# seanwood/gcc-nmf

Measured on NVIDIA H100. Metric: STFT frames/sec (1024-FFT, K=1024) full GCC-NMF pipeline, higher is better.
Workload: dtype f32

## Files before the change

gcc-nmf_b200/csrc/gcc_tc.cu:

```cuda
#include <algorithm>

#include "common.cuh"
#include "tma_gemm_host.cuh"

namespace {

using namespace tgemm_host;

inline float margin_factor(int F) {
  const double per_value = 3.0 / 262144.0 + (1.0 + 3.0 * F / 16.0) / 16777216.0;
  return (float)(2.5 * per_value);
}

__global__ void __launch_bounds__(256)
build_gcc_planes_kernel(const float2* __restrict__ coh, int F, int T, const double2* __restrict__ E, int D, bf16* __restrict__ G, int64_t pitch,
                        int64_t plane) {
  __shared__ float2 Cs[64][33];
  const int f0 = blockIdx.x * 64, t0 = blockIdx.y * 32;
  const int lane = threadIdx.x & 31, w = threadIdx.x >> 5;
  for (int i = w; i < 64; i += 8) {
    const int f = f0 + i, t = t0 + lane;
    Cs[i][lane] = (f < F && t < T) ? coh[(int64_t)f * T + t] : float2{0.f, 0.f};
  }
  __syncthreads();
// ... 26 lines not shown
    }
  }
}

__global__ void split_to_planes_kernel(const float* __restrict__ src, int64_t n, bf16* __restrict__ planes, int64_t plane) {
  const int64_t i = (int64_t)blockIdx.x * blockDim.x + threadIdx.x;
  if (i >= n) return;
  bf16 hi, lo;
  split_bf16(src[i], hi, lo);
  planes[i] = hi;
  planes[plane + i] = lo;
}

struct EpiArgmaxTile {
  static constexpr bool kTileEpilogue = true;
  static constexpr bool kRowReduce = false;
  static constexpr int kRowValues = 0;
  static constexpr bool kPrefetch = false;
  struct State {};
  struct Loaded {};
  int32_t* __restrict__ argmax;
  const float* __restrict__ colsumW;
  int2* __restrict__ list; uint4* __restrict__ candidates; int* __restrict__ count; int capacity;
  int K, T, D; float margin_factor;
  __device__ void prefetch(int, int) const {}
  __device__ void row_values(int, float*) const {}
  __device__ void elem(int, int, float, int) const {}
  __device__ void tile_epilogue(const float* __restrict__ tile, int m0, int n0, int n_valid, int) const {
    const int frames = n_valid / D;
    for (int p = threadIdx.x; p < tgemm::kBM * frames; p += blockDim.x) {
      const int ml = p & (tgemm::kBM - 1), j = p / tgemm::kBM;
      const int m = m0 + ml;
      if (m >= K) continue;
      const float* col = tile + (size_t)(j * D) * tgemm::kBM + ml;
      float best = -INFINITY, second = -INFINITY;
      int idx = 0, nan = 0;
#pragma unroll 8
      for (int d = 0; d < D; ++d) {
        const float x = col[(size_t)d * tgemm::kBM];
        if (x != x) nan = 1;
        if (x > best) { second = best; best = x; idx = d; }
        else if (x > second) second = x;
      }
      const int t = n0 / D + j;
      argmax[(int64_t)m * T + t] = idx;
      const float margin = margin_factor * colsumW[m];
      if (nan || !(best - second > margin)) {
        uint32_t bits[4] = {0u, 0u, 0u, 0u};
        for (int d = 0; d < D; ++d) {
          const float x = col[(size_t)d * tgemm::kBM];
          if (nan || !(best - x > margin)) bits[d >> 5] |= 1u << (d & 31);
        }
        const int slot = atomicAdd(count, 1);
        if (slot < capacity) {
          list[slot] = make_int2(m, t);
          candidates[slot] = make_uint4(bits[0], bits[1], bits[2], bits[3]);
        }
      }
    }
  }
};

constexpr int kPersBN = 256, kPersKB = 32, kPersStages = 4;
constexpr int kPersABytes = 2 * tgemm::kBM * kPersKB * 2;
constexpr int kPersBBytes = 2 * kPersBN * kPersKB * 2;
constexpr int kPersStageBytes = kPersABytes + kPersBBytes;
constexpr int kPersSmem = kPersStages * kPersStageBytes + 256 + 1024;
constexpr int kPersAtomBytes = 2 * kPersKB * 128;

struct ArgmaxPartial {
  float best, second;
  int idx, nan;
  __device__ void scan(float x, int d) {
    if (x != x) nan = 1;
    if (x > best) { second = best; best = x; idx = d; }
    else if (x > second) second = x;
  }
  __device__ void merge_xor(int o) {
    const float ob = __shfl_xor_sync(0xffffffffu, best, o), os = __shfl_xor_sync(0xffffffffu, second, o);
    const int oi = __shfl_xor_sync(0xffffffffu, idx, o), on = __shfl_xor_sync(0xffffffffu, nan, o);
    const bool take = ob > best || (ob == best && oi < idx);
    const float loser = take ? best : ob;
    if (take) { best = ob; idx = oi; }
// ... 585 lines not shown
```

gcc-nmf_b200/csrc/klnmf_tma.cu:

```cuda
#include <algorithm>
#include <mutex>
#include <utility>
#include <vector>

#include "common.cuh"
#include "tma_gemm_host.cuh"

void gccnmf_tmap_cache_free(gccnmf_handle* h) {
  delete h->tmaps;
  h->tmaps = nullptr;
}

namespace {

using namespace tgemm_host;

constexpr int kApplyTile = 32;

struct EpiStoreT {
  struct State {};
  struct Loaded {};
  static constexpr bool kDualN = true;
  static constexpr bool kRowReduce = false;
  static constexpr int kRowValues = 0;
  static constexpr bool kPrefetch = false;
  float* __restrict__ DT; int64_t ld, slab; int M, N; bool vec; bool streaming;
  __device__ void prefetch(int, int) const {}
  __device__ void row_values(int, float*) const {}
  __device__ void init(State&, int, const float*) const {}
  __device__ float4 row_partial(const State&) const { return make_float4(0.f, 0.f, 0.f, 0.f); }
  __device__ void row_total(int, int, float) const {}
  __device__ void elem(int m, int n, float acc, int z) const { DT[(int64_t)z * slab + (int64_t)n * ld + m] = acc; }
  __device__ Loaded load(int, int) const { return Loaded{}; }
  __device__ void store(int m, int n, const float4& acc, const Loaded&, int z, State&) const {
    const int valid = min(4, M - m);
    if (valid <= 0) return;
    if (streaming) store4_streaming(DT + (int64_t)z * slab + (int64_t)n * ld + m, acc, valid, vec);
    else store4(DT + (int64_t)z * slab + (int64_t)n * ld + m, acc, valid, vec);
  }
};

struct EpiRatioPlanes {
  struct State {};
  struct Loaded { float4 vt; };
  static constexpr bool kRowReduce = false;
  static constexpr int kRowValues = 0;
  static constexpr bool kPrefetch = false;
  static constexpr bool kDualN = true;
  static constexpr bool kPreloadOperands = true;
  const float* __restrict__ VT; bf16* __restrict__ RT; int64_t ld, plane; int M, N; bool vec;
  __device__ void prefetch(int, int) const {}
  __device__ void row_values(int, float*) const {}
  __device__ void init(State&, int, const float*) const {}
  __device__ float4 row_partial(const State&) const { return make_float4(0.f, 0.f, 0.f, 0.f); }
  __device__ void row_total(int, int, float) const {}
  __device__ void elem(int m, int n, float acc, int) const {
    bf16 hi, lo;
    split_bf16(VT[(int64_t)n * ld + m] / acc, hi, lo);
    RT[(int64_t)n * ld + m] = hi;
    RT[plane + (int64_t)n * ld + m] = lo;
  }
  __device__ Loaded load(int m, int n) const { return Loaded{load4(VT + (int64_t)n * ld + m, min(4, M - m), vec, 1.f)}; }
  __device__ void store(int m, int n, const float4& acc, const Loaded& l, int, State&) const {
    const int valid = min(4, M - m);
    if (valid <= 0) return;
    const float4 r = make_float4(__fdividef(l.vt.x, acc.x), __fdividef(l.vt.y, acc.y), __fdividef(l.vt.z, acc.z), __fdividef(l.vt.w, acc.w));
    store_planes4(RT + (int64_t)n * ld + m, plane, r, valid, vec);
  }
};

struct EpiUpdateH {
  struct State { float4 rden, rsum; };
  struct Loaded { float4 old; };
  static constexpr bool kRowReduce = true;
  static constexpr int kRowValues = 1;
  static constexpr bool kPrefetch = true;
  __device__ void prefetch(int m, int n) const {
    if (m < M) tgemm::prefetch_l2(HT + (int64_t)n * ld + m);
  }
  float* __restrict__ HT; bf16* __restrict__ HTp; const float* __restrict__ colsum_part; const float* __restrict__ sumsq_part;
  float* __restrict__ rowsum_part; float alpha, eps; int64_t ld, plane; int M, N; int slots; bool vec;
  __device__ void row_values(int m, float* v) const {
    v[0] = 1.f;
// ... 978 lines not shown
```

gcc-nmf_b200/csrc/tma_gemm.cuh:

```cuda
#pragma once
#include <cuda.h>
#include <cuda_bf16.h>
#include <cuda_runtime.h>

#include <cstdint>
#include <type_traits>

#include "gmma_ptx.cuh"

namespace tgemm {

using gmma::mbar_init;
using gmma::mbar_wait;
using gmma::smem_u32;

constexpr int kBM = 128;
constexpr int kMmaWarpgroups = 2;
constexpr int kAuxWarps = 3;
constexpr int kThreads = (1 + kMmaWarpgroups) * 128;
constexpr int kColumnsInFlight = 8;
constexpr int kMaxRowValues = 4;
constexpr int kSmemBudget = 216 * 1024;

__device__ __forceinline__ void mbar_arrive_expect_tx(uint32_t bar, uint32_t bytes) {
  asm volatile("mbarrier.arrive.expect_tx.shared::cta.b64 _, [%0], %1;" ::"r"(bar), "r"(bytes) : "memory");
}
__device__ __forceinline__ void tma_load_3d(uint32_t dst, const CUtensorMap* map, uint32_t bar, int c0, int c1, int c2) {
  asm volatile(
      "cp.async.bulk.tensor.3d.shared::cluster.global.mbarrier::complete_tx::bytes [%0], [%1, {%3, %4, %5}], [%2];"
      ::"r"(dst), "l"(reinterpret_cast<uint64_t>(map)), "r"(bar), "r"(c0), "r"(c1), "r"(c2)
      : "memory");
}
template <bool MULTICAST>
__device__ __forceinline__ void tma_load_3d_mc(uint32_t dst, const CUtensorMap* map, uint32_t bar, int c0, int c1, int c2, uint16_t mask) {
  if (MULTICAST) {
    asm volatile(
        "cp.async.bulk.tensor.3d.shared::cluster.global.mbarrier::complete_tx::bytes.multicast::cluster [%0], [%1, {%3, %4, %5}], [%2], %6;"
        ::"r"(dst), "l"(reinterpret_cast<uint64_t>(map)), "r"(bar), "r"(c0), "r"(c1), "r"(c2), "h"(mask)
        : "memory");
  } else {
    tma_load_3d(dst, map, bar, c0, c1, c2);
  }
}
__device__ __forceinline__ void cluster_sync() {
  asm volatile("barrier.cluster.arrive.release.aligned;" ::: "memory");
  asm volatile("barrier.cluster.wait.acquire.aligned;" ::: "memory");
}
__device__ __forceinline__ float4 ld_cluster_f32x4(const float* local, uint32_t rank) {
  uint32_t remote;
  asm volatile("mapa.shared::cluster.u32 %0, %1, %2;" : "=r"(remote) : "r"(gmma::smem_u32(local)), "r"(rank));
  float4 v;
  asm volatile("ld.shared::cluster.v4.f32 {%0, %1, %2, %3}, [%4];" : "=f"(v.x), "=f"(v.y), "=f"(v.z), "=f"(v.w) : "r"(remote) : "memory");
  return v;
}
__device__ __forceinline__ void tma_prefetch_descriptor(const CUtensorMap* map) {
// ... 18 lines not shown
  const uint32_t hw[4] = {h.x, h.y, h.z, h.w}, lw[4] = {l.x, l.y, l.z, l.w};
#pragma unroll
  for (int i = 0; i < 4; ++i) {
    out[2 * i] = __uint_as_float(hw[i] << 16) + __uint_as_float(lw[i] << 16);
    out[2 * i + 1] = __uint_as_float(hw[i] & 0xFFFF0000u) + __uint_as_float(lw[i] & 0xFFFF0000u);
  }
}

struct PeerSignal {
  unsigned* counters[8];
  int world;
};
__device__ __forceinline__ void signal_peers(const PeerSignal& sig) {
  for (int r = 0; r < sig.world; ++r) asm volatile("red.relaxed.sys.global.add.u32 [%0], %1;" ::"l"(sig.counters[r]), "r"(1u) : "memory");
}

struct PlaneGemmArgs {
  int M, N, Kc;
  int m_tiles;
  int tail_rows;
  int tail_cols;
  int kblocks_per_split;
  int preload;
  int m_fastest;
  int z_cluster;
  const __nv_bfloat16* A; int64_t a_plane, lda;
  const __nv_bfloat16* B; int64_t b_plane, ldb;
  unsigned* done_counter;
  PeerSignal signal;
  unsigned long long* timing;
};


template <int BN, int KB, bool A_MN, bool B_MN, int NACC = 1>
struct Config {
  static_assert(KB == 32 || KB == 64, "k-block of 32 (SWIZZLE_64B K-major rows) or 64 (SWIZZLE_128B)");
  static_assert(BN % 8 == 0 && BN >= 16 && BN * NACC <= 256, "wgmma N (= BN, or 2 BN in the dual-N loop)");
  static constexpr int kAAtoms = kBM / 64;
  static constexpr int kBAtoms = (BN + 63) / 64;
  static constexpr int kAtomBytes = 2 * KB * 128;
  static constexpr int kABytes = 2 * kBM * KB * 2;
  static constexpr int kBBytes = B_MN ? kBAtoms * kAtomBytes : 2 * BN * KB * 2;
  static constexpr int kStageBytes = kABytes + kBBytes;
  static_assert(kABytes % 1024 == 0 && kBBytes % 1024 == 0, "operand blocks must keep 1024-byte alignment");
  static constexpr int kStagesRaw = kSmemBudget / kStageBytes;
  static constexpr int kStages = kStagesRaw > 8 ? 8 : kStagesRaw;
  static_assert(kStages >= 2, "tile too large for a 2-stage pipeline");
  static constexpr int kAccCols = BN * NACC;
  static constexpr int kBarrierBytes = 256;
  static constexpr int kScratchBytes = kMaxRowValues * kBM * 4 + (kThreads / 32) * 32 * 16;
  static constexpr int kTotal = kStages * kStageBytes + kBarrierBytes + kScratchBytes + 1024;
  static_assert(kStages * kStageBytes >= BN * kBM * 4, "the epilogue stages the accumulator tile in the pipeline buffers");
  static_assert(kTotal <= 227 * 1024, "shared memory per CTA");
};

template <int N, int KB, bool A_MN, bool B_MN, bool DUAL>
__device__ __forceinline__ void mma_kblock(float (&acc)[N / 2], uint32_t a_base, uint32_t b_base, uint32_t b_lo_off) {
  constexpr uint32_t kAtom = 2 * KB * 128;
  constexpr uint32_t a_lo_off = A_MN ? KB * 128 : kBM * KB * 2;
  constexpr uint32_t a_step = A_MN ? 2048u : 32u, b_step = B_MN ? 2048u : 32u;
  constexpr uint32_t kKSbo = 8 * KB * 2;
  constexpr uint32_t kKSwizzle = (KB == 32) ? gmma::kSwizzle64B : gmma::kSwizzle128B;
  auto desc = [&](uint32_t addr, bool mn) {
    return mn ? gmma::make_desc(addr, kAtom, 1024, gmma::kSwizzle128B) : gmma::make_desc(addr, 16, kKSbo, kKSwizzle);
  };
#pragma unroll
  for (int kk = 0; kk < KB / 16; ++kk) {
    const uint32_t a_addr = a_base + kk * a_step, b_addr = b_base + kk * b_step;
    const uint64_t a_hi = desc(a_addr, A_MN), a_lo = desc(a_addr + a_lo_off, A_MN);
    const uint64_t b_hi = desc(b_addr, B_MN), b_lo = desc(b_addr + b_lo_off, B_MN);
    if constexpr (DUAL) {
      if (kk > 0) gmma::wgmma_fence();
      gmma::Wgmma<N / 2>::template mma<A_MN, B_MN>(reinterpret_cast<float(&)[N / 4]>(acc), a_lo, b_hi);
      gmma::wgmma_fence();
      gmma::Wgmma<N>::template mma<A_MN, B_MN>(acc, a_hi, b_hi);
      (void)b_lo;
    } else {
      gmma::Wgmma<N>::template mma<A_MN, B_MN>(acc, a_lo, b_hi);
      gmma::Wgmma<N>::template mma<A_MN, B_MN>(acc, a_hi, b_lo);
      gmma::Wgmma<N>::template mma<A_MN, B_MN>(acc, a_hi, b_hi);
    }
  }
}

template <class E, class = void>
struct has_tile_epilogue { static constexpr bool value = false; };
template <class E>
struct has_tile_epilogue<E, decltype((void)E::kTileEpilogue)> { static constexpr bool value = E::kTileEpilogue; };

template <class E, class = void>
struct wants_preload { static constexpr bool value = false; };
template <class E>
struct wants_preload<E, decltype((void)E::kPreloadOperands)> { static constexpr bool value = E::kPreloadOperands; };

template <class E, class = void>
struct wants_dual_n { static constexpr bool value = false; };
template <class E>
struct wants_dual_n<E, decltype((void)E::kDualN)> { static constexpr bool value = E::kDualN; };

template <int BN, int KB, bool A_MN, bool B_MN, int CN, int CM, class Epilogue>
__global__ void __launch_bounds__(kThreads, 1)
plane_gemm_kernel(const __grid_constant__ CUtensorMap map_a, const __grid_constant__ CUtensorMap map_b, PlaneGemmArgs args, Epilogue epi) {
  constexpr bool DUAL = wants_dual_n<Epilogue>::value && !B_MN && 2 * BN <= 256;
  using C = Config<BN, KB, A_MN, B_MN, DUAL ? 2 : 1>;
  constexpr int kCluster = CN * CM;
  static_assert((CN == 1 || CN == 2) && (CM == 1 || CM == 2), "cluster of CN n-tiles x CM m-tiles");
  static_assert(A_MN || (kBM / CN) % 8 == 0, "A row slices keep the swizzle atoms whole");
  static_assert(B_MN || (BN / CM) % 8 == 0, "B row slices keep the swizzle atoms whole");
  extern __shared__ unsigned char smem_dyn[];
  unsigned char* smem = reinterpret_cast<unsigned char*>((reinterpret_cast<uintptr_t>(smem_dyn) + 1023) & ~uintptr_t(1023));

  const int tid = threadIdx.x, warp = tid >> 5, lane = tid & 31;
  const bool mf = args.m_fastest != 0;
  const int tile_n = mf ? (int)blockIdx.y : (int)blockIdx.x;
  const int tile_m = mf ? (int)blockIdx.x : (int)blockIdx.y;
  const int z = blockIdx.z;
  const int n0 = tile_n * BN;
  const int total_kblocks = (args.Kc + KB - 1) / KB;
  const int kb_begin = z * args.kblocks_per_split;
  const int kb_end = min(total_kblocks, kb_begin + args.kblocks_per_split);
  const int num_kb = max(0, kb_end - kb_begin);
  const int cx = (!mf && CN > 1) ? (int)(blockIdx.x % CN) : 0;
  const int cy = (CM > 1) ? tile_m % CM : 0;
  const uint16_t mask_row = (uint16_t)(((1u << CN) - 1u) << (CN * cy));
  const uint16_t mask_col = (uint16_t)((CM > 1 ? ((1u << cx) | (1u << (cx + CN))) : (1u << cx)));

  uint64_t* bars = reinterpret_cast<uint64_t*>(smem + C::kStages * C::kStageBytes);
  uint64_t* full = bars;
  uint64_t* empty = bars + C::kStages;
  float* rowvals = reinterpret_cast<float*>(smem + C::kStages * C::kStageBytes + C::kBarrierBytes);
  float4* red = reinterpret_cast<float4*>(rowvals + kMaxRowValues * kBM);
  float* tile = reinterpret_cast<float*>(smem);
  const int m0 = tile_m * kBM;

  const int cta_linear = blockIdx.x + gridDim.x * (blockIdx.y + gridDim.y * blockIdx.z);
  if (args.timing && tid == 0) {
    args.timing[cta_linear * 8 + 0] = globaltimer_ns();
    args.timing[cta_linear * 8 + 1] = clock64();
  }
  if (tid == 0) {
    for (int s = 0; s < C::kStages; ++s) {
      mbar_init(smem_u32(&full[s]), 1);
      mbar_init(smem_u32(&empty[s]), kMmaWarpgroups * (CN + CM - 1));
    }
    gmma::fence_barrier_init();
    tma_prefetch_descriptor(&map_a);
    tma_prefetch_descriptor(&map_b);
  }
  if (kCluster > 1) cluster_sync();
  else __syncthreads();
  pdl_launch_dependents();
  pdl_wait_prior_grids();

  constexpr int kWarpsAll = kThreads / 32;
  constexpr int kLoadedWords = (int)((sizeof(typename Epilogue::Loaded) + 3) / 4);
  constexpr bool kPreloads = wants_preload<Epilogue>::value && !has_tile_epilogue<Epilogue>::value && !std::is_empty<typename Epilogue::Loaded>::value;
  constexpr int kPreCap = 64 / (kLoadedWords > 0 ? kLoadedWords : 1);
  constexpr int kPre = kPreloads ? ((BN + kWarpsAll - 1) / kWarpsAll < kPreCap ? (BN + kWarpsAll - 1) / kWarpsAll : kPreCap) : 0;
  typename Epilogue::Loaded pre[kPre > 0 ? kPre : 1];
  auto preload = [&]() {
    if constexpr (kPre > 0) {
      if (!args.preload) return;
      const int n_valid = min(BN, args.N - n0);
#pragma unroll
      for (int u = 0; u < kPre; ++u) {
        const int cc = warp + kWarpsAll * u;
        if (cc < n_valid) pre[u] = epi.load(m0 + 4 * lane, n0 + cc);
      }
    }
  };

  if (warp == 0) {
    if (lane == 0) {
      for (int i = 0; i < num_kb; ++i) {
        const int s = i % C::kStages;
        const uint32_t use = i / C::kStages;
        if (use > 0) mbar_wait(smem_u32(&empty[s]), (use - 1) & 1);
        const uint32_t bar = smem_u32(&full[s]);
        const uint32_t a_dst = smem_u32(smem + (size_t)s * C::kStageBytes), b_dst = a_dst + C::kABytes;
        const int k0 = (kb_begin + i) * KB;
        mbar_arrive_expect_tx(bar, C::kStageBytes);
        if (A_MN) {
#pragma unroll
          for (int a = 0; a < C::kAAtoms; ++a)
            if (a % CN == cx) tma_load_3d_mc<(CN > 1)>(a_dst + a * C::kAtomBytes, &map_a, bar, m0 + 64 * a, k0, 0, mask_row);
        } else {
          constexpr int kRows = kBM / CN;
#pragma unroll
          for (int p = 0; p < 2; ++p)
            tma_load_3d_mc<(CN > 1)>(a_dst + p * (kBM * KB * 2) + cx * (kRows * KB * 2), &map_a, bar, k0, m0 + cx * kRows, p, mask_row);
        }
        if (B_MN) {
#pragma unroll
          for (int a = 0; a < C::kBAtoms; ++a)
            if (a % CM == cy) tma_load_3d_mc<(CM > 1)>(b_dst + a * C::kAtomBytes, &map_b, bar, n0 + 64 * a, k0, 0, mask_col);
        } else {
          constexpr int kRows = BN / CM;
#pragma unroll
          for (int p = 0; p < 2; ++p)
            tma_load_3d_mc<(CM > 1)>(b_dst + p * (BN * KB * 2) + cy * (kRows * KB * 2), &map_b, bar, k0, n0 + cy * kRows, p, mask_col);
        }
      }
      if (args.timing) args.timing[cta_linear * 8 + 4] = clock64();
    }
    __syncwarp();
    preload();
  } else if (warp < 4) {
    const int e = warp - 1;
    if (Epilogue::kRowValues > 0) {
      for (int r = e * 32 + lane; r < kBM; r += kAuxWarps * 32) {
        float rv[Epilogue::kRowValues > 0 ? Epilogue::kRowValues : 1];
        epi.row_values(m0 + r, rv);
#pragma unroll
        for (int i = 0; i < Epilogue::kRowValues; ++i) rowvals[i * kBM + r] = rv[i];
      }
    }
    if (Epilogue::kPrefetch) {
      const int n_valid = min(BN, args.N - n0);
      if ((lane & 7) == 0)
        for (int c = e; c < n_valid; c += kAuxWarps) epi.prefetch(m0 + 4 * lane, n0 + c);
    }
    if (!A_MN && !B_MN && args.tail_rows > 0) {
      const bool z_red = kCluster == 1 && args.z_cluster > 1;
      const int k_begin = z_red ? 0 : kb_begin * KB, k_end = z_red ? args.Kc : min(args.Kc, kb_end * KB);
      const int tcols = z_red ? (((args.tail_cols + args.z_cluster - 1) / args.z_cluster) + 1) & ~1 : args.tail_cols;
      const int c_begin = n0 + (z_red ? tile_m * args.z_cluster + z : tile_m) * tcols;
      const int c_end = min(min(args.N, n0 + BN), c_begin + tcols);
      constexpr int kRound = 32 * kAuxWarps;
      for (int m = args.m_tiles * kBM; m < args.M; ++m) {
        const __nv_bfloat16* a_hi = args.A + (int64_t)m * args.lda;
        const __nv_bfloat16* a_lo = a_hi + args.a_plane;
#pragma unroll 1
        for (int c_round = c_begin; c_round < c_end; c_round += kRound) {
          float keep = 0.f;
#pragma unroll 1
          for (int i = 0; i < 16; ++i) {
            const int n = c_round + 2 * (e + i * kAuxWarps);
            if (n >= c_end) break;
            const bool two = n + 1 < c_end;
            const __nv_bfloat16* b_hi = args.B + (int64_t)n * args.ldb;
            const __nv_bfloat16* b_lo = b_hi + args.b_plane;
            const int64_t next = two ? args.ldb : 0;
            float acc0 = 0.f, acc1 = 0.f;
#pragma unroll 4
            for (int k = k_begin + 8 * lane; k < k_end; k += 256) {
              float a[8], b0[8], b1[8];
              load_planes8(a_hi + k, a_lo + k, a);
              load_planes8(b_hi + k, b_lo + k, b0);
              load_planes8(b_hi + next + k, b_lo + next + k, b1);
#pragma unroll
              for (int j = 0; j < 8; ++j) { acc0 = fmaf(a[j], b0[j], acc0); acc1 = fmaf(a[j], b1[j], acc1); }
            }
            for (int o = 16; o > 0; o >>= 1) { acc0 += __shfl_xor_sync(0xffffffffu, acc0, o); acc1 += __shfl_xor_sync(0xffffffffu, acc1, o); }
            if (lane == 2 * i) keep = acc0;
            if (lane == 2 * i + 1) keep = acc1;
          }
          const int n_mine = c_round + 2 * (e + (lane >> 1) * kAuxWarps) + (lane & 1);
          if (n_mine < c_end) epi.elem(m, n_mine, keep, z_red ? 0 : z);
        }
      }
    }
    preload();
  } else {
    const int g = (warp >> 2) - 1;
    const int wt = tid & 127;
    float acc[C::kAccCols / 2];
#pragma unroll
    for (int j = 0; j < C::kAccCols / 2; ++j) acc[j] = 0.f;
    const uint32_t a_slab = A_MN ? (uint32_t)(g * C::kAtomBytes) : (uint32_t)(g * 64 * KB * 2);
    constexpr uint32_t b_lo_off = B_MN ? KB * 128 : BN * KB * 2;
    const uint16_t mask_release = mask_row | mask_col;
    auto release = [&](int s) {
      if (wt == 0) {
        if (kCluster > 1) {
          for (uint32_t r = 0; r < (uint32_t)kCluster; ++r)
            if (mask_release & (1u << r)) gmma::mbar_arrive_cluster(smem_u32(&empty[s]), r);
        } else {
          gmma::mbar_arrive(smem_u32(&empty[s]));
        }
      }
    };
    for (int i = 0; i < num_kb; ++i) {
      const int s = i % C::kStages;
      mbar_wait(smem_u32(&full[s]), (i / C::kStages) & 1);
      if (args.timing && i == 0 && tid == 128) args.timing[cta_linear * 8 + 2] = clock64();
      const uint32_t a_base = smem_u32(smem + (size_t)s * C::kStageBytes), b_base = a_base + C::kABytes;
      gmma::fence_regs(acc);
      gmma::wgmma_fence();
      mma_kblock<C::kAccCols, KB, A_MN, B_MN, DUAL>(acc, a_base + a_slab, b_base, b_lo_off);
      gmma::wgmma_commit();
      gmma::fence_regs(acc);
      gmma::wgmma_wait<1>();
      if (i > 0) release((i - 1) % C::kStages);
    }
    gmma::wgmma_wait<0>();
    gmma::fence_regs(acc);
    if (num_kb > 0) release((num_kb - 1) % C::kStages);
    if (args.timing && tid == 128) args.timing[cta_linear * 8 + 3] = clock64();
    asm volatile("bar.sync 1, %0;" ::"n"(kMmaWarpgroups * 128) : "memory");
    if (args.timing && tid == 128) args.timing[cta_linear * 8 + 5] = clock64();
    const int r0 = 64 * g + 16 * (wt >> 5) + ((wt & 31) >> 2);
    const int c0 = 2 * (wt & 3);
#pragma unroll
    for (int j = 0; j < BN / 2; ++j) {
      const int col = 8 * (j >> 2) + c0 + (j & 1), row = r0 + 8 * ((j >> 1) & 1);
      float v = acc[j];
      if constexpr (DUAL) v += acc[j + BN / 2];
      tile[(size_t)col * kBM + row] = v;
    }
    preload();
  }
  __syncthreads();
  const int zc = (kCluster == 1 && !has_tile_epilogue<Epilogue>::value) ? args.z_cluster : 0;
  if (zc > 1) cluster_sync();
  if constexpr (has_tile_epilogue<Epilogue>::value) {
    epi.tile_epilogue(tile, m0, n0, min(BN, args.N - n0), z);
    if (args.timing && tid == 64) args.timing[cta_linear * 8 + 6] = clock64();
  } else {
    constexpr int kWarps = kThreads / 32;
    const int m_first = m0 + 4 * lane;
    typename Epilogue::State st;
    epi.init(st, m_first, rowvals + 4 * lane);
    int n_valid = min(BN, args.N - n0);
    constexpr int U = kColumnsInFlight;
    int c_first = warp;
    if (zc > 1) {
      const int per = (n_valid + zc - 1) / zc;
      c_first = z * per + warp;
      n_valid = min(n_valid, (z + 1) * per);
    }
    if constexpr (kPre > 0) {
      if (args.preload && zc <= 1) {
#pragma unroll
        for (int u = 0; u < kPre; ++u) {
          const int cc = warp + kWarps * u;
          if (cc < n_valid) {
            const float4 acc = *reinterpret_cast<const float4*>(tile + (size_t)cc * kBM + 4 * lane);
            epi.store(m_first, n0 + cc, acc, pre[u], z, st);
          }
        }
        c_first = warp + kWarps * kPre;
      }
    }
#pragma unroll 1
    for (int c = c_first; c < n_valid; c += kWarps * U) {
      typename Epilogue::Loaded loaded[U];
#pragma unroll
      for (int u = 0; u < U; ++u) {
        const int cc = c + kWarps * u;
        if (cc < n_valid) loaded[u] = epi.load(m_first, n0 + cc);
      }
      if (zc > 1) {
        float4 sum[U];
#pragma unroll
        for (int u = 0; u < U; ++u) {
          const int cc = c + kWarps * u;
          const float* src = tile + (size_t)(cc < n_valid ? cc : 0) * kBM + 4 * lane;
          sum[u] = z == 0 ? *reinterpret_cast<const float4*>(src) : ld_cluster_f32x4(src, 0);
        }
        for (int r = 1; r < zc; ++r) {
          float4 t[U];
#pragma unroll
          for (int u = 0; u < U; ++u) {
            const int cc = c + kWarps * u;
            const float* src = tile + (size_t)(cc < n_valid ? cc : 0) * kBM + 4 * lane;
            t[u] = r == z ? *reinterpret_cast<const float4*>(src) : ld_cluster_f32x4(src, (uint32_t)r);
          }
#pragma unroll
          for (int u = 0; u < U; ++u) { sum[u].x += t[u].x; sum[u].y += t[u].y; sum[u].z += t[u].z; sum[u].w += t[u].w; }
        }
#pragma unroll
        for (int u = 0; u < U; ++u) {
          const int cc = c + kWarps * u;
          if (cc < n_valid) epi.store(m_first, n0 + cc, sum[u], loaded[u], 0, st);
        }
      } else {
#pragma unroll
        for (int u = 0; u < U; ++u) {
          const int cc = c + kWarps * u;
          if (cc < n_valid) {
            const float4 acc = *reinterpret_cast<const float4*>(tile + (size_t)cc * kBM + 4 * lane);
            epi.store(m_first, n0 + cc, acc, loaded[u], z, st);
          }
        }
      }
    }
    if constexpr (Epilogue::kRowReduce) {
      red[warp * 32 + lane] = epi.row_partial(st);
      __syncthreads();
      if (tid < kBM) {
        const float* r = reinterpret_cast<const float*>(red);
        float sum = 0.f;
#pragma unroll
        for (int w = 0; w < kWarps; ++w) sum += r[w * kBM + tid];
        epi.row_total(m0 + tid, tile_n, sum);
      }
    }
    if (args.timing && tid == 64) args.timing[cta_linear * 8 + 6] = clock64();
  }
  if (kCluster > 1 || zc > 1) cluster_sync();
  else __syncthreads();
  if (args.signal.world > 0 && tid == 0) {
    __threadfence();
    const unsigned prev = atomicAdd(args.done_counter, 1u);
    if (prev == gridDim.x * gridDim.y * gridDim.z - 1) {
      *args.done_counter = 0;
      __threadfence();
      signal_peers(args.signal);
    }
  }
  if (args.timing && tid == 0) args.timing[cta_linear * 8 + 7] = globaltimer_ns();
}

}
// ... 1 lines not shown
```

gcc-nmf_b200/csrc/tma_gemm_host.cuh:

```cuda
#pragma once
#include <algorithm>
#include <mutex>
#include <utility>
#include <vector>

#include "common.cuh"
#include "tma_gemm.cuh"

namespace tgemm_host {

using tgemm::PlaneGemmArgs;
using tgemm::split_bf16;
typedef __nv_bfloat16 bf16;

constexpr int kKB = 32;
constexpr int kTailRowsMax = 8;
constexpr int kMaxSplits = 8;

typedef CUresult (*EncodeTiledFn)(CUtensorMap*, CUtensorMapDataType, cuuint32_t, void*, const cuuint64_t*, const cuuint64_t*,
                                  const cuuint32_t*, const cuuint32_t*, CUtensorMapInterleave, CUtensorMapSwizzle,
                                  CUtensorMapL2promotion, CUtensorMapFloatOOBfill);

inline EncodeTiledFn encode_tiled_fn() {
  static EncodeTiledFn fn = nullptr;
  static std::once_flag once;
  std::call_once(once, [] {
    void* p = nullptr;
    cudaDriverEntryPointQueryResult q;
    if (cudaGetDriverEntryPoint("cuTensorMapEncodeTiled", &p, cudaEnableDefault, &q) == cudaSuccess && q == cudaDriverEntryPointSuccess)
      fn = reinterpret_cast<EncodeTiledFn>(p);
  });
  return fn;
}

struct TmapKey {
  const void* base;
  uint64_t inner, rows, pitch_bytes, plane_bytes;
  uint32_t box_inner, box_rows, box_planes;
  bool operator==(const TmapKey& o) const {
    return base == o.base && inner == o.inner && rows == o.rows && pitch_bytes == o.pitch_bytes && plane_bytes == o.plane_bytes &&
           box_inner == o.box_inner && box_rows == o.box_rows && box_planes == o.box_planes;
  }
};

}

struct gccnmf_tmap_cache {
  std::vector<std::pair<tgemm_host::TmapKey, CUtensorMap>> entries;
};

namespace tgemm_host {

inline int get_tmap(gccnmf_handle* h, const bf16* base, uint64_t inner, uint64_t rows, uint64_t pitch_elems, uint64_t plane_elems,
             uint32_t box_inner, uint32_t box_rows, uint32_t box_planes, CUtensorMap* out) {
  if (!h->tmaps) h->tmaps = new gccnmf_tmap_cache();
  const TmapKey key{base, inner, rows, pitch_elems * 2, plane_elems * 2, box_inner, box_rows, box_planes};
  for (auto& e : h->tmaps->entries)
    if (e.first == key) { *out = e.second; return 0; }
  EncodeTiledFn encode = encode_tiled_fn();
  if (!encode) return gccnmf_fail(h, GCCNMF_ERR_CUDA, "cuTensorMapEncodeTiled is not available from the driver");
  if ((reinterpret_cast<uintptr_t>(base) & 15) || (key.pitch_bytes & 15) || (key.plane_bytes & 15))
    return gccnmf_fail(h, GCCNMF_ERR_INVALID_ARGUMENT, "tensor map: base / pitch / plane stride must be 16-byte aligned");
  const cuuint64_t dims[3] = {inner, rows, 2};
  const cuuint64_t strides[2] = {key.pitch_bytes, key.plane_bytes};
  const cuuint32_t box[3] = {box_inner, box_rows, box_planes};
  const cuuint32_t elem_strides[3] = {1, 1, 1};
  const CUtensorMapSwizzle swz = (box_inner * 2 == 128) ? CU_TENSOR_MAP_SWIZZLE_128B : CU_TENSOR_MAP_SWIZZLE_64B;
  CUtensorMap m;
  const CUresult r = encode(&m, CU_TENSOR_MAP_DATA_TYPE_BFLOAT16, 3, const_cast<bf16*>(base), dims, strides, box, elem_strides,
                            CU_TENSOR_MAP_INTERLEAVE_NONE, swz, CU_TENSOR_MAP_L2_PROMOTION_L2_128B, CU_TENSOR_MAP_FLOAT_OOB_FILL_NONE);
  if (r != CUDA_SUCCESS) return gccnmf_fail(h, GCCNMF_ERR_CUDA, "cuTensorMapEncodeTiled failed with CUresult %d", (int)r);
  if (h->tmaps->entries.size() > 256) h->tmaps->entries.clear();
  h->tmaps->entries.emplace_back(key, m);
  *out = m;
  return 0;
}

inline int tmap_kmajor(gccnmf_handle* h, const bf16* planes, int rows, int kc, int64_t pitch, int64_t plane, int box_rows, CUtensorMap* out) {
  return get_tmap(h, planes, (uint64_t)kc, (uint64_t)rows, (uint64_t)pitch, (uint64_t)plane, kKB, (uint32_t)box_rows, 1, out);
}
inline int tmap_mnmajor(gccnmf_handle* h, const bf16* planes, int mn, int kc, int64_t pitch, int64_t plane, CUtensorMap* out) {
  return get_tmap(h, planes, (uint64_t)mn, (uint64_t)kc, (uint64_t)pitch, (uint64_t)plane, 64, kKB, 2, out);
}

template <class... KArgs, class... Args>
int launch_ex(gccnmf_handle* h, const char* name, void (*kernel)(KArgs...), dim3 grid, dim3 block, size_t smem, void* stream, bool pdl,
              dim3 cluster, Args&&... args) {
  cudaLaunchConfig_t cfg{};
  cfg.gridDim = grid;
  cfg.blockDim = block;
  cfg.dynamicSmemBytes = smem;
  cfg.stream = (cudaStream_t)stream;
  cudaLaunchAttribute attr[3];
  int n = 0;
  if (h->l2_window_bytes > 0) {
    attr[n].id = cudaLaunchAttributeAccessPolicyWindow;
    attr[n].val.accessPolicyWindow.base_ptr = const_cast<void*>(h->l2_window_base);
    attr[n].val.accessPolicyWindow.num_bytes = h->l2_window_bytes;
    attr[n].val.accessPolicyWindow.hitRatio = 1.0f;
    attr[n].val.accessPolicyWindow.hitProp = cudaAccessPropertyPersisting;
    attr[n].val.accessPolicyWindow.missProp = cudaAccessPropertyNormal;
    ++n;
  }
  if (pdl) {
    attr[n].id = cudaLaunchAttributeProgrammaticStreamSerialization;
    attr[n].val.programmaticStreamSerializationAllowed = 1;
    ++n;
  }
  if (cluster.x * cluster.y * cluster.z > 1) {
    attr[n].id = cudaLaunchAttributeClusterDimension;
    attr[n].val.clusterDim.x = cluster.x;
    attr[n].val.clusterDim.y = cluster.y;
    attr[n].val.clusterDim.z = cluster.z;
    ++n;
  }
// ... 39 lines not shown
}
__device__ __forceinline__ void store4_streaming(float* p, const float4& v, int valid, bool vec) {
  if (vec && valid == 4) { __stcs(reinterpret_cast<float4*>(p), v); return; }
  if (valid > 0) __stcs(p, v.x);
  if (valid > 1) __stcs(p + 1, v.y);
  if (valid > 2) __stcs(p + 2, v.z);
  if (valid > 3) __stcs(p + 3, v.w);
}
__device__ __forceinline__ void store4(float* p, const float4& v, int valid, bool vec) {
  if (vec && valid == 4) { *reinterpret_cast<float4*>(p) = v; return; }
  if (valid > 0) p[0] = v.x;
  if (valid > 1) p[1] = v.y;
  if (valid > 2) p[2] = v.z;
  if (valid > 3) p[3] = v.w;
}

struct Operand {
  const bf16* planes;
  int64_t pitch, plane;
  bool mn_major;
};

struct GemmShape {
  int M, N, Kc, splits, m_tiles, n_tiles, tail_rows;
  bool m_fastest;
  int z_cluster;
  unsigned* done_counter;
  tgemm::PeerSignal signal;
};

template <int BN, bool A_MN, bool B_MN, int CN, int CM, class Epi>
struct PlaneGemmInstance {
  static constexpr bool kDual = tgemm::wants_dual_n<Epi>::value && !B_MN && 2 * BN <= 256;
  using C = tgemm::Config<BN, kKB, A_MN, B_MN, kDual ? 2 : 1>;
  static int max_clusters(gccnmf_handle* h, int* out) {
    static int cached_per_device[kGccnmfMaxDevices];
    int& slot = cached_per_device[h->device % kGccnmfMaxDevices];
    int cached = slot - 1;
    if (cached < 0) {
      auto kernel = tgemm::plane_gemm_kernel<BN, kKB, A_MN, B_MN, CN, CM, Epi>;
      GCCNMF_CHECK_CUDA(h, cudaFuncSetAttribute(kernel, cudaFuncAttributeMaxDynamicSharedMemorySize, C::kTotal));
      if (CN * CM == 1) {
        cached = h->sm_count;
      } else {
        cudaLaunchConfig_t cfg{};
        cfg.gridDim = dim3(CN * 64, CM * 64, 1);
        cfg.blockDim = dim3(tgemm::kThreads);
        cfg.dynamicSmemBytes = C::kTotal;
        cudaLaunchAttribute attr[1];
        attr[0].id = cudaLaunchAttributeClusterDimension;
        attr[0].val.clusterDim.x = CN; attr[0].val.clusterDim.y = CM; attr[0].val.clusterDim.z = 1;
        cfg.attrs = attr;
        cfg.numAttrs = 1;
        int n = 0;
        GCCNMF_CHECK_CUDA(h, cudaOccupancyMaxActiveClusters(&n, kernel, &cfg));
        cached = n;
      }
      slot = cached + 1;
    }
    *out = cached;
    return 0;
  }
  static int max_z_clusters(gccnmf_handle* h, int S, int* out) {
    static int cached_per_device[kGccnmfMaxDevices][9];
    if (S < 2 || S > 8 || CN * CM != 1) { *out = 0; return 0; }
    int& slot = cached_per_device[h->device % kGccnmfMaxDevices][S];
    if (slot == 0) {
      int unused;
      if (int st = max_clusters(h, &unused)) return st;
      auto kernel = tgemm::plane_gemm_kernel<BN, kKB, A_MN, B_MN, CN, CM, Epi>;
      cudaLaunchConfig_t cfg{};
      cfg.gridDim = dim3(16, 16, S);
      cfg.blockDim = dim3(tgemm::kThreads);
      cfg.dynamicSmemBytes = C::kTotal;
      cudaLaunchAttribute attr[1];
      attr[0].id = cudaLaunchAttributeClusterDimension;
      attr[0].val.clusterDim.x = 1; attr[0].val.clusterDim.y = 1; attr[0].val.clusterDim.z = S;
      cfg.attrs = attr;
      cfg.numAttrs = 1;
      int n = 0;
      const cudaError_t err = cudaOccupancyMaxActiveClusters(&n, kernel, &cfg);
      if (err != cudaSuccess) { (void)cudaGetLastError(); n = 0; }
      slot = n + 1;
    }
    *out = slot - 1;
    return 0;
  }
  static int launch(gccnmf_handle* h, const Operand& A, const Operand& B, const GemmShape& g, const Epi& epi, unsigned long long* timing, void* stream) {
    auto kernel = tgemm::plane_gemm_kernel<BN, kKB, A_MN, B_MN, CN, CM, Epi>;
    int unused;
    if (int st = max_clusters(h, &unused)) return st;
    CUtensorMap map_a, map_b;
    if (int st = A_MN ? tmap_mnmajor(h, A.planes, g.M, g.Kc, A.pitch, A.plane, &map_a)
                      : tmap_kmajor(h, A.planes, g.M, g.Kc, A.pitch, A.plane, tgemm::kBM / CN, &map_a)) return st;
    if (int st = B_MN ? tmap_mnmajor(h, B.planes, g.N, g.Kc, B.pitch, B.plane, &map_b)
                      : tmap_kmajor(h, B.planes, g.N, g.Kc, B.pitch, B.plane, BN / CM, &map_b)) return st;
    PlaneGemmArgs args{};
    args.M = g.M; args.N = g.N; args.Kc = g.Kc;
    args.m_tiles = g.m_tiles;
    args.tail_rows = g.tail_rows;
    args.tail_cols = (((BN + g.m_tiles - 1) / g.m_tiles) + 1) & ~1;
    const int total_kb = (g.Kc + kKB - 1) / kKB;
    args.kblocks_per_split = (total_kb + g.splits - 1) / g.splits;
    args.A = A.planes; args.a_plane = A.plane; args.lda = A.pitch;
    args.B = B.planes; args.b_plane = B.plane; args.ldb = B.pitch;
    args.timing = timing;
    args.preload = (g.z_cluster > 1) ? 0 : (h->gemm_preload & 1);
    const bool mf = g.m_fastest;
    args.m_fastest = mf ? 1 : 0;
    args.z_cluster = (CN * CM == 1 && g.z_cluster > 1) ? g.z_cluster : 0;
    args.done_counter = g.done_counter;
    args.signal = g.signal;
    const dim3 grid = mf ? dim3(g.m_tiles, g.n_tiles, g.splits) : dim3(g.n_tiles, g.m_tiles, g.splits);
    if (!timing && h->debug_timing) {
      args.timing = h->debug_timing + h->debug_timing_cursor;
      h->debug_timing_cursor += (size_t)grid.x * grid.y * grid.z * 8;
    }
    return launch_ex(h, "plane_gemm_kernel", kernel, grid, dim3(tgemm::kThreads), (size_t)C::kTotal, stream, h->nmf_pdl,
                     args.z_cluster > 1 ? dim3(1, 1, args.z_cluster) : (mf ? dim3(CM, 1, 1) : dim3(CN, CM, 1)), map_a, map_b, args, epi);
  }
};

template <int BN, bool A_MN, bool B_MN, class Epi>
int launch_plane_gemm(gccnmf_handle* h, const Operand& A, const Operand& B, int M, int N, int Kc, int splits, bool simt_tail,
                      const Epi& epi, unsigned long long* timing, void* stream, bool m_fastest = false, bool prefer_pair = false) {
  GemmShape g{};
  g.M = M; g.N = N; g.Kc = Kc; g.splits = splits; g.m_fastest = m_fastest;
  const int tail = M % tgemm::kBM;
  const bool use_tail = simt_tail && !A_MN && !B_MN && tail != 0 && tail <= kTailRowsMax && M > tgemm::kBM && (M / tgemm::kBM) * 128 >= BN;
  g.m_tiles = use_tail ? M / tgemm::kBM : (M + tgemm::kBM - 1) / tgemm::kBM;
  g.tail_rows = use_tail ? tail : 0;
  g.n_tiles = (N + BN - 1) / BN;
  const int ctas = g.n_tiles * g.m_tiles * splits;
  const bool pair = h->gemm_pair > 0 || (h->gemm_pair < 0 && prefer_pair);
  const int order_share_b[4][2] = {{1, 2}, {1, 1}, {1, 1}, {1, 1}}, order_none[4][2] = {{1, 1}, {1, 1}, {1, 1}, {1, 1}};
  const int order_forced[4][2] = {{2, 2}, {1, 2}, {2, 1}, {1, 1}};
  const int (*order)[2] = h->gemm_cluster >= 0 ? order_forced : (pair ? order_share_b : order_none);
  for (int i = 0; i < 4; ++i) {
    const int cn = order[i][0], cm = order[i][1];
    if (h->gemm_cluster >= 0 && h->gemm_cluster != 10 * cn + cm && !(cn == 1 && cm == 1)) continue;
    if (g.n_tiles % cn != 0 || g.m_tiles % cm != 0) continue;
    if (m_fastest && cn != 1) continue;
    int resident = 0;
#define GCCNMF_TRY_CLUSTER(CN_, CM_)                                                                                         \
    if constexpr (B_MN || (BN / CM_) % 8 == 0)               \
    if (cn == CN_ && cm == CM_) {                                                                                            \
      if (int st = PlaneGemmInstance<BN, A_MN, B_MN, CN_, CM_, Epi>::max_clusters(h, &resident)) return st;                  \
                  \
      if (cn * cm == 1 || (resident > 0 && (ctas > h->sm_count || resident * cn * cm >= ctas)))                                \
          return PlaneGemmInstance<BN, A_MN, B_MN, CN_, CM_, Epi>::launch(h, A, B, g, epi, timing, stream);                  \
    }
    GCCNMF_TRY_CLUSTER(2, 2)
// ... 64 lines not shown
```

Baseline: 135,600.

## Load epilogue operand tile via TMA into shared memory and pad accumulator tile

Replaces the register-based epilogue operand preload (per-warp global loads of VT) with a TMA bulk load of the whole fp32 operand tile into a dedicated shared-memory region. The load is issued by the producer thread after the mainloop, or after the tile store when preload is off. The epilogue then waits on an mbarrier before reading operands. The accumulator staging tile also gets a padded pitch (kBM+4) to reduce shared-memory bank conflicts. The cost is extra shared memory, which can reduce pipeline stages, plus a more general tensor-map cache key.

Result: faster. 139,700, median of 6 (+3.0%).

```diff
diff --git a/gcc-nmf_b200/csrc/gcc_tc.cu b/gcc-nmf_b200/csrc/gcc_tc.cu
--- a/gcc-nmf_b200/csrc/gcc_tc.cu
+++ b/gcc-nmf_b200/csrc/gcc_tc.cu
@@ -82,12 +82,12 @@
       const int ml = p & (tgemm::kBM - 1), j = p / tgemm::kBM;
       const int m = m0 + ml;
       if (m >= K) continue;
-      const float* col = tile + (size_t)(j * D) * tgemm::kBM + ml;
+      const float* col = tile + (size_t)(j * D) * tgemm::kTilePitch + ml;
       float best = -INFINITY, second = -INFINITY;
       int idx = 0, nan = 0;
 #pragma unroll 8
       for (int d = 0; d < D; ++d) {
-        const float x = col[(size_t)d * tgemm::kBM];
+        const float x = col[(size_t)d * tgemm::kTilePitch];
         if (x != x) nan = 1;
         if (x > best) { second = best; best = x; idx = d; }
         else if (x > second) second = x;
@@ -98,7 +98,7 @@
       if (nan || !(best - second > margin)) {
         uint32_t bits[4] = {0u, 0u, 0u, 0u};
         for (int d = 0; d < D; ++d) {
-          const float x = col[(size_t)d * tgemm::kBM];
+          const float x = col[(size_t)d * tgemm::kTilePitch];
           if (nan || !(best - x > margin)) bits[d >> 5] |= 1u << (d & 31);
         }
         const int slot = atomicAdd(count, 1);
diff --git a/gcc-nmf_b200/csrc/klnmf_tma.cu b/gcc-nmf_b200/csrc/klnmf_tma.cu
--- a/gcc-nmf_b200/csrc/klnmf_tma.cu
+++ b/gcc-nmf_b200/csrc/klnmf_tma.cu
@@ -47,8 +47,9 @@
   static constexpr int kRowValues = 0;
   static constexpr bool kPrefetch = false;
   static constexpr bool kDualN = true;
-  static constexpr bool kPreloadOperands = true;
+  static constexpr bool kTmaOperand = true;
   const float* __restrict__ VT; bf16* __restrict__ RT; int64_t ld, plane; int M, N; bool vec;
+  tgemm::TmaOperand tma_operand() const { return {VT, ld}; }
   __device__ void prefetch(int, int) const {}
   __device__ void row_values(int, float*) const {}
   __device__ void init(State&, int, const float*) const {}
diff --git a/gcc-nmf_b200/csrc/tma_gemm.cuh b/gcc-nmf_b200/csrc/tma_gemm.cuh
--- a/gcc-nmf_b200/csrc/tma_gemm.cuh
+++ b/gcc-nmf_b200/csrc/tma_gemm.cuh
@@ -4,7 +4,6 @@
 #include <cuda_runtime.h>
 
 #include <cstdint>
-#include <type_traits>
 
 #include "gmma_ptx.cuh"
 
@@ -21,6 +20,8 @@
 constexpr int kColumnsInFlight = 8;
 constexpr int kMaxRowValues = 4;
 constexpr int kSmemBudget = 216 * 1024;
+constexpr int kTilePitch = kBM + 4;
+constexpr int kMinStagesWithOperand = 4;
 
 __device__ __forceinline__ void mbar_arrive_expect_tx(uint32_t bar, uint32_t bytes) {
   asm volatile("mbarrier.arrive.expect_tx.shared::cta.b64 _, [%0], %1;" ::"r"(bar), "r"(bytes) : "memory");
@@ -105,7 +106,7 @@
 };
 
 
-template <int BN, int KB, bool A_MN, bool B_MN, int NACC = 1>
+template <int BN, int KB, bool A_MN, bool B_MN, int NACC = 1, bool TMA_OP = false>
 struct Config {
   static_assert(KB == 32 || KB == 64, "k-block of 32 (SWIZZLE_64B K-major rows) or 64 (SWIZZLE_128B)");
   static_assert(BN % 8 == 0 && BN >= 16 && BN * NACC <= 256, "wgmma N (= BN, or 2 BN in the dual-N loop)");
@@ -116,14 +117,16 @@
   static constexpr int kBBytes = B_MN ? kBAtoms * kAtomBytes : 2 * BN * KB * 2;
   static constexpr int kStageBytes = kABytes + kBBytes;
   static_assert(kABytes % 1024 == 0 && kBBytes % 1024 == 0, "operand blocks must keep 1024-byte alignment");
-  static constexpr int kStagesRaw = kSmemBudget / kStageBytes;
+  static constexpr bool kOperandInSmem = TMA_OP && (kSmemBudget - BN * kBM * 4) / kStageBytes >= kMinStagesWithOperand;
+  static constexpr int kOperandBytes = kOperandInSmem ? BN * kBM * 4 : 0;
+  static constexpr int kStagesRaw = (kSmemBudget - kOperandBytes) / kStageBytes;
   static constexpr int kStages = kStagesRaw > 8 ? 8 : kStagesRaw;
   static_assert(kStages >= 2, "tile too large for a 2-stage pipeline");
   static constexpr int kAccCols = BN * NACC;
   static constexpr int kBarrierBytes = 256;
   static constexpr int kScratchBytes = kMaxRowValues * kBM * 4 + (kThreads / 32) * 32 * 16;
-  static constexpr int kTotal = kStages * kStageBytes + kBarrierBytes + kScratchBytes + 1024;
-  static_assert(kStages * kStageBytes >= BN * kBM * 4, "the epilogue stages the accumulator tile in the pipeline buffers");
+  static constexpr int kTotal = kStages * kStageBytes + kOperandBytes + kBarrierBytes + kScratchBytes + 1024;
+  static_assert(kStages * kStageBytes >= BN * kTilePitch * 4, "the epilogue stages the accumulator tile in the pipeline buffers");
   static_assert(kTotal <= 227 * 1024, "shared memory per CTA");
 };
 
@@ -161,10 +164,14 @@
 template <class E>
 struct has_tile_epilogue<E, decltype((void)E::kTileEpilogue)> { static constexpr bool value = E::kTileEpilogue; };
 
+struct TmaOperand {
+  const float* base;
+  int64_t ld;
+};
 template <class E, class = void>
-struct wants_preload { static constexpr bool value = false; };
+struct has_tma_operand { static constexpr bool value = false; };
 template <class E>
-struct wants_preload<E, decltype((void)E::kPreloadOperands)> { static constexpr bool value = E::kPreloadOperands; };
+struct has_tma_operand<E, decltype((void)E::kTmaOperand)> { static constexpr bool value = E::kTmaOperand; };
 
 template <class E, class = void>
 struct wants_dual_n { static constexpr bool value = false; };
@@ -173,9 +180,11 @@
 
 template <int BN, int KB, bool A_MN, bool B_MN, int CN, int CM, class Epilogue>
 __global__ void __launch_bounds__(kThreads, 1)
-plane_gemm_kernel(const __grid_constant__ CUtensorMap map_a, const __grid_constant__ CUtensorMap map_b, PlaneGemmArgs args, Epilogue epi) {
+plane_gemm_kernel(const __grid_constant__ CUtensorMap map_a, const __grid_constant__ CUtensorMap map_b,
+                  const __grid_constant__ CUtensorMap map_op, PlaneGemmArgs args, Epilogue epi) {
   constexpr bool DUAL = wants_dual_n<Epilogue>::value && !B_MN && 2 * BN <= 256;
-  using C = Config<BN, KB, A_MN, B_MN, DUAL ? 2 : 1>;
+  using C = Config<BN, KB, A_MN, B_MN, DUAL ? 2 : 1, has_tma_operand<Epilogue>::value>;
+  constexpr bool kOpSmem = C::kOperandInSmem;
   constexpr int kCluster = CN * CM;
   static_assert((CN == 1 || CN == 2) && (CM == 1 || CM == 2), "cluster of CN n-tiles x CM m-tiles");
   static_assert(A_MN || (kBM / CN) % 8 == 0, "A row slices keep the swizzle atoms whole");
@@ -198,10 +207,12 @@
   const uint16_t mask_row = (uint16_t)(((1u << CN) - 1u) << (CN * cy));
   const uint16_t mask_col = (uint16_t)((CM > 1 ? ((1u << cx) | (1u << (cx + CN))) : (1u << cx)));
 
-  uint64_t* bars = reinterpret_cast<uint64_t*>(smem + C::kStages * C::kStageBytes);
+  const float* opnd = reinterpret_cast<const float*>(smem + C::kStages * C::kStageBytes);
+  uint64_t* bars = reinterpret_cast<uint64_t*>(smem + C::kStages * C::kStageBytes + C::kOperandBytes);
   uint64_t* full = bars;
   uint64_t* empty = bars + C::kStages;
-  float* rowvals = reinterpret_cast<float*>(smem + C::kStages * C::kStageBytes + C::kBarrierBytes);
+  uint64_t* op_full = bars + 2 * C::kStages;
+  float* rowvals = reinterpret_cast<float*>(smem + C::kStages * C::kStageBytes + C::kOperandBytes + C::kBarrierBytes);
   float4* red = reinterpret_cast<float4*>(rowvals + kMaxRowValues * kBM);
   float* tile = reinterpret_cast<float*>(smem);
   const int m0 = tile_m * kBM;
@@ -216,30 +227,21 @@
       mbar_init(smem_u32(&full[s]), 1);
       mbar_init(smem_u32(&empty[s]), kMmaWarpgroups * (CN + CM - 1));
     }
+    if (kOpSmem) mbar_init(smem_u32(op_full), 1);
     gmma::fence_barrier_init();
     tma_prefetch_descriptor(&map_a);
     tma_prefetch_descriptor(&map_b);
+    if (kOpSmem) tma_prefetch_descriptor(&map_op);
   }
   if (kCluster > 1) cluster_sync();
   else __syncthreads();
   pdl_launch_dependents();
   pdl_wait_prior_grids();
 
-  constexpr int kWarpsAll = kThreads / 32;
-  constexpr int kLoadedWords = (int)((sizeof(typename Epilogue::Loaded) + 3) / 4);
-  constexpr bool kPreloads = wants_preload<Epilogue>::value && !has_tile_epilogue<Epilogue>::value && !std::is_empty<typename Epilogue::Loaded>::value;
-  constexpr int kPreCap = 64 / (kLoadedWords > 0 ? kLoadedWords : 1);
-  constexpr int kPre = kPreloads ? ((BN + kWarpsAll - 1) / kWarpsAll < kPreCap ? (BN + kWarpsAll - 1) / kWarpsAll : kPreCap) : 0;
-  typename Epilogue::Loaded pre[kPre > 0 ? kPre : 1];
-  auto preload = [&]() {
-    if constexpr (kPre > 0) {
-      if (!args.preload) return;
-      const int n_valid = min(BN, args.N - n0);
-#pragma unroll
-      for (int u = 0; u < kPre; ++u) {
-        const int cc = warp + kWarpsAll * u;
-        if (cc < n_valid) pre[u] = epi.load(m0 + 4 * lane, n0 + cc);
-      }
+  auto load_operand = [&]() {
+    if constexpr (kOpSmem) {
+      mbar_arrive_expect_tx(smem_u32(op_full), (uint32_t)C::kOperandBytes);
+      tma_load_3d(smem_u32(opnd), &map_op, smem_u32(op_full), m0, n0, 0);
     }
   };
 
@@ -275,9 +277,8 @@
         }
       }
       if (args.timing) args.timing[cta_linear * 8 + 4] = clock64();
-    }
-    __syncwarp();
-    preload();
+      if (args.preload) load_operand();
+    }
   } else if (warp < 4) {
     const int e = warp - 1;
     if (Epilogue::kRowValues > 0) {
@@ -333,7 +334,6 @@
         }
       }
     }
-    preload();
   } else {
     const int g = (warp >> 2) - 1;
     const int wt = tid & 127;
@@ -379,11 +379,11 @@
       const int col = 8 * (j >> 2) + c0 + (j & 1), row = r0 + 8 * ((j >> 1) & 1);
       float v = acc[j];
       if constexpr (DUAL) v += acc[j + BN / 2];
-      tile[(size_t)col * kBM + row] = v;
-    }
-    preload();
+      tile[(size_t)col * kTilePitch + row] = v;
+    }
   }
   __syncthreads();
+  if (!args.preload && tid == 0) load_operand();
   const int zc = (kCluster == 1 && !has_tile_epilogue<Epilogue>::value) ? args.z_cluster : 0;
   if (zc > 1) cluster_sync();
   if constexpr (has_tile_epilogue<Epilogue>::value) {
@@ -402,33 +402,25 @@
       c_first = z * per + warp;
       n_valid = min(n_valid, (z + 1) * per);
     }
-    if constexpr (kPre > 0) {
-      if (args.preload && zc <= 1) {
-#pragma unroll
-        for (int u = 0; u < kPre; ++u) {
-          const int cc = warp + kWarps * u;
-          if (cc < n_valid) {
-            const float4 acc = *reinterpret_cast<const float4*>(tile + (size_t)cc * kBM + 4 * lane);
-            epi.store(m_first, n0 + cc, acc, pre[u], z, st);
-          }
-        }
-        c_first = warp + kWarps * kPre;
-      }
-    }
+    if (kOpSmem) mbar_wait(smem_u32(op_full), 0);
 #pragma unroll 1
     for (int c = c_first; c < n_valid; c += kWarps * U) {
       typename Epilogue::Loaded loaded[U];
 #pragma unroll
       for (int u = 0; u < U; ++u) {
         const int cc = c + kWarps * u;
-        if (cc < n_valid) loaded[u] = epi.load(m_first, n0 + cc);
+        if constexpr (kOpSmem) {
+          if (cc < n_valid) loaded[u] = typename Epilogue::Loaded{*reinterpret_cast<const float4*>(opnd + (size_t)cc * kBM + 4 * lane)};
+        } else {
+          if (cc < n_valid) loaded[u] = epi.load(m_first, n0 + cc);
+        }
       }
       if (zc > 1) {
         float4 sum[U];
 #pragma unroll
         for (int u = 0; u < U; ++u) {
           const int cc = c + kWarps * u;
-          const float* src = tile + (size_t)(cc < n_valid ? cc : 0) * kBM + 4 * lane;
+          const float* src = tile + (size_t)(cc < n_valid ? cc : 0) * kTilePitch + 4 * lane;
           sum[u] = z == 0 ? *reinterpret_cast<const float4*>(src) : ld_cluster_f32x4(src, 0);
         }
         for (int r = 1; r < zc; ++r) {
@@ -436,7 +428,7 @@
 #pragma unroll
           for (int u = 0; u < U; ++u) {
             const int cc = c + kWarps * u;
-            const float* src = tile + (size_t)(cc < n_valid ? cc : 0) * kBM + 4 * lane;
+            const float* src = tile + (size_t)(cc < n_valid ? cc : 0) * kTilePitch + 4 * lane;
             t[u] = r == z ? *reinterpret_cast<const float4*>(src) : ld_cluster_f32x4(src, (uint32_t)r);
           }
 #pragma unroll
@@ -452,7 +444,7 @@
         for (int u = 0; u < U; ++u) {
           const int cc = c + kWarps * u;
           if (cc < n_valid) {
-            const float4 acc = *reinterpret_cast<const float4*>(tile + (size_t)cc * kBM + 4 * lane);
+            const float4 acc = *reinterpret_cast<const float4*>(tile + (size_t)cc * kTilePitch + 4 * lane);
             epi.store(m_first, n0 + cc, acc, loaded[u], z, st);
           }
         }
diff --git a/gcc-nmf_b200/csrc/tma_gemm_host.cuh b/gcc-nmf_b200/csrc/tma_gemm_host.cuh
--- a/gcc-nmf_b200/csrc/tma_gemm_host.cuh
+++ b/gcc-nmf_b200/csrc/tma_gemm_host.cuh
@@ -35,11 +35,14 @@
 
 struct TmapKey {
   const void* base;
-  uint64_t inner, rows, pitch_bytes, plane_bytes;
+  CUtensorMapDataType dtype;
+  CUtensorMapSwizzle swizzle;
+  uint64_t inner, rows, planes, pitch_bytes, plane_bytes;
   uint32_t box_inner, box_rows, box_planes;
   bool operator==(const TmapKey& o) const {
-    return base == o.base && inner == o.inner && rows == o.rows && pitch_bytes == o.pitch_bytes && plane_bytes == o.plane_bytes &&
-           box_inner == o.box_inner && box_rows == o.box_rows && box_planes == o.box_planes;
+    return base == o.base && dtype == o.dtype && swizzle == o.swizzle && inner == o.inner && rows == o.rows && planes == o.planes &&
+           pitch_bytes == o.pitch_bytes && plane_bytes == o.plane_bytes && box_inner == o.box_inner && box_rows == o.box_rows &&
+           box_planes == o.box_planes;
   }
 };
 
@@ -51,24 +54,25 @@
 
 namespace tgemm_host {
 
-inline int get_tmap(gccnmf_handle* h, const bf16* base, uint64_t inner, uint64_t rows, uint64_t pitch_elems, uint64_t plane_elems,
-             uint32_t box_inner, uint32_t box_rows, uint32_t box_planes, CUtensorMap* out) {
+inline int get_tmap(gccnmf_handle* h, const void* base, CUtensorMapDataType dtype, CUtensorMapSwizzle swizzle, uint64_t inner,
+                    uint64_t rows, uint64_t planes, uint64_t pitch_elems, uint64_t plane_elems, uint32_t box_inner, uint32_t box_rows,
+                    uint32_t box_planes, CUtensorMap* out) {
   if (!h->tmaps) h->tmaps = new gccnmf_tmap_cache();
-  const TmapKey key{base, inner, rows, pitch_elems * 2, plane_elems * 2, box_inner, box_rows, box_planes};
+  const uint64_t elem_bytes = dtype == CU_TENSOR_MAP_DATA_TYPE_FLOAT32 ? 4 : 2;
+  const TmapKey key{base, dtype, swizzle, inner, rows, planes, pitch_elems * elem_bytes, plane_elems * elem_bytes, box_inner, box_rows, box_planes};
   for (auto& e : h->tmaps->entries)
     if (e.first == key) { *out = e.second; return 0; }
   EncodeTiledFn encode = encode_tiled_fn();
   if (!encode) return gccnmf_fail(h, GCCNMF_ERR_CUDA, "cuTensorMapEncodeTiled is not available from the driver");
   if ((reinterpret_cast<uintptr_t>(base) & 15) || (key.pitch_bytes & 15) || (key.plane_bytes & 15))
     return gccnmf_fail(h, GCCNMF_ERR_INVALID_ARGUMENT, "tensor map: base / pitch / plane stride must be 16-byte aligned");
-  const cuuint64_t dims[3] = {inner, rows, 2};
+  const cuuint64_t dims[3] = {inner, rows, planes};
   const cuuint64_t strides[2] = {key.pitch_bytes, key.plane_bytes};
   const cuuint32_t box[3] = {box_inner, box_rows, box_planes};
   const cuuint32_t elem_strides[3] = {1, 1, 1};
-  const CUtensorMapSwizzle swz = (box_inner * 2 == 128) ? CU_TENSOR_MAP_SWIZZLE_128B : CU_TENSOR_MAP_SWIZZLE_64B;
   CUtensorMap m;
-  const CUresult r = encode(&m, CU_TENSOR_MAP_DATA_TYPE_BFLOAT16, 3, const_cast<bf16*>(base), dims, strides, box, elem_strides,
-                            CU_TENSOR_MAP_INTERLEAVE_NONE, swz, CU_TENSOR_MAP_L2_PROMOTION_L2_128B, CU_TENSOR_MAP_FLOAT_OOB_FILL_NONE);
+  const CUresult r = encode(&m, dtype, 3, const_cast<void*>(base), dims, strides, box, elem_strides,
+                            CU_TENSOR_MAP_INTERLEAVE_NONE, swizzle, CU_TENSOR_MAP_L2_PROMOTION_L2_128B, CU_TENSOR_MAP_FLOAT_OOB_FILL_NONE);
   if (r != CUDA_SUCCESS) return gccnmf_fail(h, GCCNMF_ERR_CUDA, "cuTensorMapEncodeTiled failed with CUresult %d", (int)r);
   if (h->tmaps->entries.size() > 256) h->tmaps->entries.clear();
   h->tmaps->entries.emplace_back(key, m);
@@ -77,10 +81,16 @@
 }
 
 inline int tmap_kmajor(gccnmf_handle* h, const bf16* planes, int rows, int kc, int64_t pitch, int64_t plane, int box_rows, CUtensorMap* out) {
-  return get_tmap(h, planes, (uint64_t)kc, (uint64_t)rows, (uint64_t)pitch, (uint64_t)plane, kKB, (uint32_t)box_rows, 1, out);
+  return get_tmap(h, planes, CU_TENSOR_MAP_DATA_TYPE_BFLOAT16, CU_TENSOR_MAP_SWIZZLE_64B, (uint64_t)kc, (uint64_t)rows, 2,
+                  (uint64_t)pitch, (uint64_t)plane, kKB, (uint32_t)box_rows, 1, out);
 }
 inline int tmap_mnmajor(gccnmf_handle* h, const bf16* planes, int mn, int kc, int64_t pitch, int64_t plane, CUtensorMap* out) {
-  return get_tmap(h, planes, (uint64_t)mn, (uint64_t)kc, (uint64_t)pitch, (uint64_t)plane, 64, kKB, 2, out);
+  return get_tmap(h, planes, CU_TENSOR_MAP_DATA_TYPE_BFLOAT16, CU_TENSOR_MAP_SWIZZLE_128B, (uint64_t)mn, (uint64_t)kc, 2,
+                  (uint64_t)pitch, (uint64_t)plane, 64, kKB, 2, out);
+}
+inline int tmap_f32_tile(gccnmf_handle* h, const float* base, int M, int N, int64_t ld, int box_cols, CUtensorMap* out) {
+  return get_tmap(h, base, CU_TENSOR_MAP_DATA_TYPE_FLOAT32, CU_TENSOR_MAP_SWIZZLE_NONE, (uint64_t)M, (uint64_t)N, 1, (uint64_t)ld,
+                  (uint64_t)ld * (uint64_t)N, (uint32_t)tgemm::kBM, (uint32_t)box_cols, 1, out);
 }
 
 template <class... KArgs, class... Args>
@@ -186,7 +196,7 @@
 template <int BN, bool A_MN, bool B_MN, int CN, int CM, class Epi>
 struct PlaneGemmInstance {
   static constexpr bool kDual = tgemm::wants_dual_n<Epi>::value && !B_MN && 2 * BN <= 256;
-  using C = tgemm::Config<BN, kKB, A_MN, B_MN, kDual ? 2 : 1>;
+  using C = tgemm::Config<BN, kKB, A_MN, B_MN, kDual ? 2 : 1, tgemm::has_tma_operand<Epi>::value>;
   static int max_clusters(gccnmf_handle* h, int* out) {
     static int cached_per_device[kGccnmfMaxDevices];
     int& slot = cached_per_device[h->device % kGccnmfMaxDevices];
@@ -249,6 +259,11 @@
                       : tmap_kmajor(h, A.planes, g.M, g.Kc, A.pitch, A.plane, tgemm::kBM / CN, &map_a)) return st;
     if (int st = B_MN ? tmap_mnmajor(h, B.planes, g.N, g.Kc, B.pitch, B.plane, &map_b)
                       : tmap_kmajor(h, B.planes, g.N, g.Kc, B.pitch, B.plane, BN / CM, &map_b)) return st;
+    CUtensorMap map_op{};
+    if constexpr (C::kOperandInSmem) {
+      const tgemm::TmaOperand op = epi.tma_operand();
+      if (int st = tmap_f32_tile(h, op.base, g.M, g.N, op.ld, BN, &map_op)) return st;
+    }
     PlaneGemmArgs args{};
     args.M = g.M; args.N = g.N; args.Kc = g.Kc;
     args.m_tiles = g.m_tiles;
@@ -259,7 +274,7 @@
     args.A = A.planes; args.a_plane = A.plane; args.lda = A.pitch;
     args.B = B.planes; args.b_plane = B.plane; args.ldb = B.pitch;
     args.timing = timing;
-    args.preload = (g.z_cluster > 1) ? 0 : (h->gemm_preload & 1);
+    args.preload = h->gemm_preload & 1;
     const bool mf = g.m_fastest;
     args.m_fastest = mf ? 1 : 0;
     args.z_cluster = (CN * CM == 1 && g.z_cluster > 1) ? g.z_cluster : 0;
@@ -271,7 +286,7 @@
       h->debug_timing_cursor += (size_t)grid.x * grid.y * grid.z * 8;
     }
     return launch_ex(h, "plane_gemm_kernel", kernel, grid, dim3(tgemm::kThreads), (size_t)C::kTotal, stream, h->nmf_pdl,
-                     args.z_cluster > 1 ? dim3(1, 1, args.z_cluster) : (mf ? dim3(CM, 1, 1) : dim3(CN, CM, 1)), map_a, map_b, args, epi);
+                     args.z_cluster > 1 ? dim3(1, 1, args.z_cluster) : (mf ? dim3(CM, 1, 1) : dim3(CN, CM, 1)), map_a, map_b, map_op, args, epi);
   }
 };
 
```
